# zengyan-97/X2-VLM

Measured on AMD Instinct MI355X. Metric: image-text pairs/sec (fwd+bwd) X2VLM-base 224px bs=64/GPU, higher is better.
Workload: dtype bf16

## Files before the change

### include/x2vlm_hip.h

```cpp
#ifndef X2VLM_HIP_H
#define X2VLM_HIP_H
#include <stdint.h>
#ifdef __cplusplus
extern "C" {
#endif

const char* x2_last_error(void);
int x2_abi_version(void);
int x2_device_cus(void);
int x2_tune(int key, int value);
int x2_tune_get(int key);

int x2_gemm_nt(const void* A, const void* B, void* C, int M, int N, int K, int lda, int ldb, int ldc,
               const float* bias, const float* gamma, const float* resid, int ldr, void* aux, int ldaux,
               int act, int out_f32, unsigned drop_thr16, unsigned drop_seed, float drop_scale, const unsigned* drop_epoch,
               const float* rowscale, float* colsum, void* stream);

int x2_gemm_nt_dgelu_colparts(const void* A, const void* B, void* C, int M, int N, int K, int lda, int ldb, int ldc,
                              const void* aux, int ldaux, float* colparts, int* nrows_out, void* stream);
int x2_gemm_nt_splitk(const void* A, const void* B, float* C, int M, int N, int K, int lda, int ldb, int ldc,
                      int slices, float* ws, long ws_floats, void* stream);

int x2_gemm_tn_grouped(const int64_t* problems, int count, int accumulate, int split, float* ws, long ws_floats,
                       void* stream);
int x2_tn_plan(const int64_t* shapes, int count, int cus, long ws_floats, int* windows, int max_windows, int* launches, int max_launches,
               int* n_windows, int* n_launches);
int x2_gemm_tn_queue(const int64_t* problems, int count, int accumulate, float* ws, long ws_floats, int first_launch, int n_launches,
                     void* stream);

typedef struct X2AttnArgs {
  const void *Q, *K, *V, *O, *dO;
  void *Out, *dQ, *dK, *dV, *dS;
  float *LSE, *Delta;
  long q_bs, q_rs, k_bs, k_rs, v_bs, v_rs, o_bs, o_rs;
  long dq_bs, dq_rs, dk_bs, dk_rs, dv_bs, dv_rs, do_bs, do_rs;
  int B, Bkv, H, Lq, Lk;
  float scale;
  const float* bias;  int bias_ld;
  const float* biasT; int biasT_ld;
  const float* mask;  int mask_ld;
  const int* kv_idx;
  const int* seq_off; const int* seq_ids;
  int ds_ld;
  unsigned drop_thr16, drop_seed; float drop_scale;
  int dbg;
  int head_dim;
  const unsigned* drop_epoch;
  int grid_nx, grid_ny, grid_nz, grid_map;
  int phase;
  float* ws; long ws_floats;
  float* colsum_ws;
} X2AttnArgs;
int x2_attn_fwd(const X2AttnArgs* args, void* stream);
int x2_attn_bwd(const X2AttnArgs* args, void* stream);
int x2_attn_bwd_one_pass(const X2AttnArgs* args);

int x2_layernorm_fwd(const float* x, const float* w, const float* b, void* y_bf16, float* y_f32, float* mean,
                     float* rstd, int rows, int D, float eps, int period, unsigned drop_thr16, unsigned drop_seed,
                     float drop_scale, const unsigned* drop_epoch, void* stream);
int x2_layernorm_bwd(const void* dy , int dy_is_bf16, const float* x, const float* mean, const float* rstd, const float* w,
                     const float* dres, float* dx, void* dx_bf16, float* dw, float* db, float* dcol, int rows, int D,
                     int period, unsigned in_thr16, unsigned in_seed, float in_scale, unsigned out_thr16,
                     unsigned out_seed, float out_scale, const unsigned* drop_epoch, float* ws ,
                     int defer, int post, const float* post_rowscale, void* stream);
int x2_colsum_bf16(const void* y, float* out, int M, int N, int ld, float* ws , int defer, void* stream);
int x2_reduce_partials(const float* part, int nblk, int nk, int width, float* o0, float* o1, float* o2, void* stream);
int x2_reduce_partials_multi(const int64_t* desc, int count, void* stream);
int x2_layerscale_finish(const int64_t* desc, int count, void* stream);
int x2_rowscale_cast_colsum(const float* dx, const float* rowscale, void* dx_bf16, float* colsum, int M, int D,
                            float* ws , int defer, void* stream);
int x2_cast_bf16(const float* src, void* dst, long n, void* stream);
int x2_cast_transpose_bf16(const float* src, void* dst, void* dstT, int R, int C, int ldt, void* stream);
int x2_cast_transpose_multi(const int64_t* desc, int count, void* stream);
int x2_copy_f32_multi(const int64_t* desc, int count, void* stream);
int x2_patchify(const float* image, void* cols, int B, int R, int ps, void* stream);
int x2_assemble_tokens(const float* patch, const float* cls, float* x, int B, int P, int D, void* stream);
int x2_assemble_tokens_bwd(const float* dx, void* dpatch_bf16, float* dcls, int B, int P, int D, void* stream);
int x2_pool_tokens(float* x, const float* w, int B, int P, int D, int bwd, void* stream);
int x2_relpos_bias(const float* table, const long* index, const long* indexT , float* bias, float* biasT, int N, int H, int ld, int ldT,
                   float scale, void* stream);
int x2_relpos_bias_bwd(const void* dS, const int* inv_off, const int* inv_pos, float* dtable, int B, int N, int H, int ld,
                       int T, float* ws, int slices, void* stream);

int x2_embed_fwd(const long* ids, const float* word, const float* pos, const float* type0, float* out, int R, int L,
                 int D, void* stream);
int x2_embed_bwd(const long* ids, const float* g, float* dword, float* dpos, float* dtype0, int R, int L, int D,
                 float* scratch, void* stream);
int x2_gather_rows(const float* src, const int* idx, float* dst, void* dst_bf16, int R, long len, void* stream);
int x2_scatter_rows(const float* src, const int* idx, float* dst, int R, int D, long len, void* stream);
int x2_linear_f32(const float* A, const float* B, float* C, const float* bias, const float* alpha_ptr, float alpha,
                  int M, int N, int K, long sam, long sak, long sbn, long sbk, long ldc, int accumulate,
                  int ksplit ,
                  float* ws , void* stream);
int x2_l2norm(const float* x, const float* dy, float* out, int R, int D, int bwd, void* stream);
int x2_ce_fwd(const float* logits, long ld, const long* labels, int R, int C, float* lse, float* loss_row, float* out2,
              void* stream);
int x2_ce_bwd(const float* logits, long ld, const long* labels, const float* lse, const float* g, const float* stat,
              float gscale, int R, int C, float* dl_f32, void* dl_bf16, long ldd, void* stream);
int x2_mlm_ce_fwd(const void* X, const void* E, const float* bias, const long* labels, int R, int Vp, int V, int Hd,
                  int ldx, int lde, float* part, float* zlab, void* stream);
int x2_ce_combine(const float* part, int chunks, const float* zlab, const long* labels, int R, float* lse, float* loss_row,
                  float* out2, void* stream);
int x2_mlm_ce_bwd(const void* X, const void* E, const float* bias, const long* labels, const float* lse, const float* g,
                  const float* stat, float gscale, int R, int Vp, int V, int Hd, int ldx, int lde, void* dl_bf16, long ldd,
                  void* stream);
int x2_mask_tokens(const long* text_ids, const long* text_atts, int B, int L, const unsigned char* is_subword, int vocab,
                   const unsigned* words, int words_ld, unsigned seed, const unsigned* epoch, double mask_prob, int max_masks,
                   double skipgram_prb, int skipgram_size, int mask_whole_word, long cls_id, long mask_id, long pad_id, long pad_mask,
                   long* text_ids_masked, long* masked_pos, long* masked_ids, void* stream);
int x2_sample_negatives(const float* sim, int n, const long* group, const float* u, int* out, void* stream);
int x2_additive_mask(const long* atts, float* out, int S, int L, int Lp, float neg, void* stream);
// ... 86 lines not shown
```

### x2-vlm_amd/_lib.py

```python
import contextlib
import ctypes as C
import os

import torch

_HERE = os.path.dirname(os.path.abspath(__file__))
LIB_PATH = os.environ.get("X2VLM_HIP_LIB") or os.path.join(_HERE, "libx2vlm_hip.so")

P, I, L, F, U = C.c_void_p, C.c_int, C.c_long, C.c_float, C.c_uint


class AttnArgs(C.Structure):
    _fields_ = [(n, P) for n in ("Q", "K", "V", "O", "dO", "Out", "dQ", "dK", "dV", "dS", "LSE", "Delta")] + \
               [(n, L) for n in ("q_bs", "q_rs", "k_bs", "k_rs", "v_bs", "v_rs", "o_bs", "o_rs",
                                 "dq_bs", "dq_rs", "dk_bs", "dk_rs", "dv_bs", "dv_rs", "do_bs", "do_rs")] + \
               [(n, I) for n in ("B", "Bkv", "H", "Lq", "Lk")] + [("scale", F)] + \
               [("bias", P), ("bias_ld", I), ("biasT", P), ("biasT_ld", I), ("mask", P), ("mask_ld", I),
                ("kv_idx", P), ("seq_off", P), ("seq_ids", P), ("ds_ld", I),
                ("drop_thr16", C.c_uint), ("drop_seed", C.c_uint), ("drop_scale", F), ("dbg", I), ("head_dim", I), ("drop_epoch", P),
                ("grid_nx", I), ("grid_ny", I), ("grid_nz", I), ("grid_map", I),
                ("phase", I), ("ws", P), ("ws_floats", L), ("colsum_ws", P)]


_SIGS = {
    "x2_gemm_nt": [P, P, P, I, I, I, I, I, I, P, P, P, I, P, I, I, I, U, U, F, P, P, P, P],
    "x2_gemm_nt_splitk": [P, P, P, I, I, I, I, I, I, I, P, L, P],
    "x2_gemm_nt_dgelu_colparts": [P, P, P, I, I, I, I, I, I, P, I, P, C.POINTER(I), P],
    "x2_gemm_tn_grouped": [P, I, I, I, P, L, P],
    "x2_gemm_tn_queue": [P, I, I, P, L, I, I, P],
    "x2_attn_fwd": [C.POINTER(AttnArgs), P],
    "x2_attn_bwd": [C.POINTER(AttnArgs), P],
    "x2_layernorm_fwd": [P, P, P, P, P, P, P, I, I, F, I, U, U, F, P, P],
    "x2_layernorm_bwd": [P, I, P, P, P, P, P, P, P, P, P, P, I, I, I, U, U, F, U, U, F, P, P, I, I, P, P],
    "x2_colsum_bf16": [P, P, I, I, I, P, I, P],
    "x2_reduce_partials": [P, I, I, I, P, P, P, P],
    "x2_reduce_partials_multi": [P, I, P],
    "x2_cast_transpose_multi": [P, I, P],
    "x2_copy_f32_multi": [P, I, P],
    "x2_layerscale_finish": [P, I, P],
    "x2_rowscale_cast_colsum": [P, P, P, P, I, I, P, I, P],
    "x2_cast_bf16": [P, P, L, P],
    "x2_cast_transpose_bf16": [P, P, P, I, I, I, P],
    "x2_patchify": [P, P, I, I, I, P],
    "x2_assemble_tokens": [P, P, P, I, I, I, P],
    "x2_assemble_tokens_bwd": [P, P, P, I, I, I, P],
    "x2_pool_tokens": [P, P, I, I, I, I, P],
    "x2_relpos_bias": [P, P, P, P, P, I, I, I, I, F, P],
    "x2_relpos_bias_bwd": [P, P, P, P, I, I, I, I, I, P, I, P],
    "x2_embed_fwd": [P, P, P, P, P, I, I, I, P],
    "x2_embed_bwd": [P, P, P, P, P, I, I, I, P, P],
    "x2_gather_rows": [P, P, P, P, I, L, P],
    "x2_scatter_rows": [P, P, P, I, I, L, P],
    "x2_linear_f32": [P, P, P, P, P, F, I, I, I, L, L, L, L, L, I, I, P, P],
    "x2_l2norm": [P, P, P, I, I, I, P],
    "x2_ce_fwd": [P, L, P, I, I, P, P, P, P],
    "x2_ce_bwd": [P, L, P, P, P, P, F, I, I, P, P, L, P],
    "x2_mlm_ce_fwd": [P, P, P, P, I, I, I, I, I, I, P, P, P],
    "x2_ce_combine": [P, I, P, P, I, P, P, P, P],
    "x2_mlm_ce_bwd": [P, P, P, P, P, P, P, F, I, I, I, I, I, I, P, L, P],
    "x2_sample_negatives": [P, I, P, P, P, P],
    "x2_mask_tokens": [P, P, I, I, P, I, P, I, U, P, C.c_double, I, C.c_double, I, I, L, L, L, L, P, P, P, P],
    "x2_additive_mask": [P, P, I, I, I, F, P],
    "x2_kv_csr": [P, I, I, P, P, P],
    "x2_tail_index": [P, P, P, P, I, I, I, I, P, P, P, P, P],
    "x2_droppath_rows": [P, U, P, I, I, I, P, P],
    "x2_frame_mean": [P, P, P, P, P, I, I, I, I, I, P],
    "x2_gelu_f32": [P, P, P, L, P],
    "x2_grad_norm": [P, I, I, F, P, P, P],
    "x2_adamw_multi": [P, I, I, P, P, I, F, F, F, P, P],
    "x2_colsum_f32": [P, P, I, I, P],
    "x2_attn_fwd_mask2d": [C.POINTER(AttnArgs), P, I, P],
    "x2_attn_bwd_mask2d": [C.POINTER(AttnArgs), P, I, P],
    "x2_additive_mask2d": [P, P, I, I, I, F, P],
    "x2_embed_fwd_pid": [P, P, P, P, P, P, I, I, P],
    "x2_embed_bwd_pid": [P, P, P, P, P, P, I, I, I, P, P],
    "x2_mlm_ls_fwd": [P, P, P, P, L, I, I, I, I, I, I, P, P, P, P, P],
    "x2_ls_combine": [P, P, I, P, P, P, P, I, I, L, F, P, P, P, P],
    "x2_mlm_ls_bwd": [P, P, P, P, P, P, P, P, F, F, L, I, I, I, I, I, I, P, L, P],
    "x2_attn_decode": [P, I, P, P, I, I, I, I, I, I, F, P],
    "x2_beam_gather": [P, P, P, I, I, I, I, I, P],
    "x2_logprob_topk": [P, I, I, I, P, I, I, I, I, I, I, P, P, P, P],
    "x2_answer_topk": [P, I, I, I, P, I, I, P, P, P],
    "x2_vqa_candidates": [P, P, P, I, I, I, I, L, P, P, P, P, I, P],
    "x2_vqa_rerank": [P, I, P, P, I, I, P, P, P, P],
    "x2_vqa_train_rows": [P, P, P, P, I, I, I, L, P, P, P, I, P, P],
    "x2_seq_loss_combine": [P, I, P, P, I, I, P, P, P, P, P],
    "x2_mlm_seq_bwd": [P, P, P, P, P, P, P, I, I, I, I, I, I, I, P, L, P],
    "x2_bbox_loss_fwd": [P, P, P, I, P, P, P],
    "x2_bbox_loss_bwd": [P, P, P, P, P, P, P, I, P, P],
    "x2_grounding_iou": [P, P, P, I, P, P, P],
    "x2_cls_tail_fwd": [P, I, P, P, P, P, P, I, I, I, F, P, P, P, P, P],
    "x2_cls_tail_bwd": [P, I, P, P, P, P, P, P, P, P, P, I, I, I, P, I, P, P, P, P, P],
    "x2_cls_accuracy": [P, P, I, I, P, P, P],
    "x2_lngelu_fwd": [P, I, P, P, I, I, F, P, I, P, P],
    "x2_lngelu_bwd": [P, I, P, I, P, P, P, I, I, P, I, P, P, P],
    "x2_soft_ce_fwd": [P, I, I, I, P, P, P, I, P, P, P, P],
    "x2_kl_ce_fwd": [P, I, P, I, I, I, P, P, P, P, P],
    "x2_soft_ce_bwd": [P, I, I, I, P, P, P, P, P, P, P, I, P, I, I, P],
    "x2_kl_ce_bwd": [P, I, P, I, I, I, P, P, P, P, I, P, I, I, P],
    "x2_cls_accuracy_rows": [P, I, P, I, I, P, P, P, P],
}
_COMM_SIGS = {
    "x2_comm_unique_id": [P],
    "x2_comm_init": [P, I, I, C.POINTER(P)],
    "x2_comm_info": [P, C.POINTER(I), C.POINTER(I)],
    "x2_comm_allreduce_bucket": [P, P, L, I, I, P, P],
    "x2_comm_allgather": [P, P, P, L, I, P, P],
    "x2_comm_broadcast": [P, P, L, I, I, P, P],
    "x2_comm_destroy": [P],
}
EXPORTS = sorted(list(_SIGS) + list(_COMM_SIGS) + ["x2_last_error", "x2_abi_version", "x2_device_cus", "x2_tune", "x2_tune_get",
                                                         "x2_attn_bwd_one_pass", "x2_tn_plan"])

_lib = None


class X2HipError(RuntimeError):
    pass


def lib():
    global _lib
    if _lib is None:
        if not os.path.exists(LIB_PATH):
            raise X2HipError("HIP extension %s not built: run `python -c 'import __graft_entry__ as g; g.build()'`"
                             % LIB_PATH)
        try:
            h = C.CDLL(LIB_PATH)
        except OSError as e:
            raise X2HipError("cannot load %s: %s" % (LIB_PATH, e))
        for name, sig in list(_SIGS.items()) + list(_COMM_SIGS.items()):
            fn = getattr(h, name)
            fn.argtypes, fn.restype = sig, I
        h.x2_last_error.restype = C.c_char_p
        h.x2_abi_version.restype = I
        h.x2_device_cus.restype = I
        h.x2_tune.argtypes, h.x2_tune.restype = [I, I], I
        h.x2_tune_get.argtypes, h.x2_tune_get.restype = [I], I
        h.x2_attn_bwd_one_pass.argtypes, h.x2_attn_bwd_one_pass.restype = [C.POINTER(AttnArgs)], I
        h.x2_tn_plan.argtypes, h.x2_tn_plan.restype = [P, I, I, L, P, I, P, I, C.POINTER(I), C.POINTER(I)], I
        for kv in filter(None, os.environ.get("X2_TUNE", "").split(",")):
            k, v = kv.split("=")
            set_tune(int(k), int(v), h)
        _lib = h
    return _lib


def set_tune(key, value, h=None):
    h = lib() if h is None else h
    if h.x2_tune(key, value) != 0:
        raise X2HipError("x2_tune(%d, %d): %s" % (key, value, h.x2_last_error().decode()))


@contextlib.contextmanager
def tuned(knobs):
    h = lib()
    with contextlib.ExitStack() as undo:
        for key, value in knobs.items():
            prev = h.x2_tune_get(key)
            if prev == -1:
                raise X2HipError("x2_tune_get(%d): no such key" % key)
            if prev != value:
                set_tune(key, value, h)
                undo.callback(set_tune, key, prev, h)
        yield


_get_device = torch._C._cuda_getDevice if hasattr(torch._C, "_cuda_getDevice") else None
_get_raw_stream = getattr(torch._C, "_cuda_getCurrentRawStream", None)


def raw_stream():
    return _get_raw_stream(_get_device())


def call(name, *args):
    h = _lib or lib()
    rc = getattr(h, name)(*args, _get_raw_stream(_get_device()))
    if rc != 0:
        raise X2HipError("%s failed (%d): %s" % (name, rc, h.x2_last_error().decode()))


def ptr(t):
    return None if t is None else t.data_ptr()
```

### x2-vlm_amd/csrc/gemm.hip

```cpp
#include "x2_common.h"
#include <algorithm>
#include <type_traits>
#include <vector>

#define BM 128
#define BN 128
#define BK 64
#define TILE_BYTES (128 * 128)
#define STAGE_BYTES (2 * TILE_BYTES)
#define GEMM_LDS_BYTES (2 * STAGE_BYTES)

struct GemmNT {
  const bf16_t* A; const bf16_t* B; void* C;
  const float* bias; const float* gamma; const float* resid; bf16_t* aux;
  int M, N, K;
  int lda, ldb, ldc, ldr, ldaux;
  int act;
  int out_f32;
  int group_m;
  DropSpec drop;
  const uint32_t* drop_epoch;
  const float* rowscale;
  float* colsum;
  int dbg;
// ... 1513 lines not shown
  const float* src = ws + (size_t)tile * 65536 + (size_t)e * 4;
  float4 o = *reinterpret_cast<const float4*>(src);
  for (int s_ = 1; s_ < split; ++s_) {
    const float4 v = *reinterpret_cast<const float4*>(src + (size_t)s_ * total_tiles * 65536);
    o.x += v.x; o.y += v.y; o.z += v.z; o.w += v.w;
  }
  if (n >= p.N || k >= p.K) return;
  float* dst = p.C + (size_t)n * p.ldc + k;
  if (g.accumulate) { const float4 c = *reinterpret_cast<float4*>(dst); o.x += c.x; o.y += c.y; o.z += c.z; o.w += c.w; }
  *reinterpret_cast<float4*>(dst) = o;
}

static int tn_parse(const char* who, const int64_t* q, int i, TNProblem& p) {
  p.A = (const bf16_t*)q[0]; p.B = (const bf16_t*)q[1]; p.C = (float*)q[2];
  p.Mc = (int)q[3]; p.N = (int)q[4]; p.K = (int)q[5]; p.lda = (int)q[6]; p.ldb = (int)q[7]; p.ldc = (int)q[8];
  p.n_ld = (int)q[9]; p.k_ld = (int)q[10];
  p.tile_begin = 0; p.tiles_k = 0; p.tile_first = 0;
  X2_REQUIRE(p.Mc > 0 && p.N > 0 && p.K > 0, "%s[%d]: empty problem", who, i);
  X2_REQUIRE(p.K % 4 == 0 && p.ldc % 4 == 0, "%s[%d]: K, ldc must be multiples of 4", who, i);
  X2_REQUIRE(p.lda % 8 == 0 && p.ldb % 8 == 0 && p.n_ld % 8 == 0 && p.k_ld % 8 == 0 && p.n_ld >= 8 && p.k_ld >= 8,
             "%s[%d]: rows must be 16-byte granular", who, i);
  X2_REQUIRE(p.n_ld <= p.lda && p.k_ld <= p.ldb, "%s[%d]: n_ld/k_ld exceed leading dims", who, i);
  return X2_OK;
}
static int tn_split_rule(int t, int min_steps, int cus, int split, bool have_ws, long ws_floats) {
  int sp = split;
  if (sp == 0) {
    double best = -1.0; sp = 1;
    for (int c = 1; c <= 4 && min_steps / c >= 16; ++c) {
      const long blocks = (long)t * c;
      const double fill = (double)blocks / (double)(((blocks + cus - 1) / cus) * cus);
      if (fill > best + 0.03) { best = fill; sp = c; }
    }
  }
  while (sp > 1 && (sp > min_steps || !have_ws || (long)sp * t * 65536 > ws_floats)) --sp;
  return sp;
}
static void tn256_launch(const GemmTNGroup& g, int t, int sp, float* ws, hipStream_t stream) {
  static bool attr = false;
  if (!attr) {
    (void)hipFuncSetAttribute(reinterpret_cast<const void*>(gemm_tn256_kernel<false>), hipFuncAttributeMaxDynamicSharedMemorySize, T2_LDS_BYTES);
    (void)hipFuncSetAttribute(reinterpret_cast<const void*>(gemm_tn256_kernel<true>), hipFuncAttributeMaxDynamicSharedMemorySize, T2_LDS_BYTES);
    attr = true;
  }
  bool ragged = false;
  for (int i = 0; i < g.count; ++i) ragged = ragged || (g.p[i].Mc % BK != 0);
  if (ragged) hipLaunchKernelGGL(gemm_tn256_kernel<true>, dim3(t, sp), dim3(512), T2_LDS_BYTES, stream, g, ws, t);
  else hipLaunchKernelGGL(gemm_tn256_kernel<false>, dim3(t, sp), dim3(512), T2_LDS_BYTES, stream, g, ws, t);
  if (sp > 1) hipLaunchKernelGGL(gemm_tn256_reduce_kernel, dim3(t * 64), dim3(256), 0, stream, g, ws, t, sp);
}

extern "C" int x2_gemm_tn_grouped(const int64_t* problems, int count, int accumulate, int split, float* ws, long ws_floats,
                                  void* stream) {
  X2_REQUIRE(count >= 1 && count <= 8, "x2_gemm_tn_grouped: count=%d not in [1,8]", count);
  X2_REQUIRE(split >= 0, "x2_gemm_tn_grouped: split=%d", split);
  GemmTNGroup g{}; g.count = count; g.accumulate = accumulate;
  int tiles256 = 0, min_steps = 1 << 30;
  bool big = g_tune[5] != 1;
  for (int i = 0; i < count; ++i) {
    TNProblem& p = g.p[i];
    if (int rc = tn_parse("x2_gemm_tn_grouped", problems + i * 11, i, p)) return rc;
    tiles256 += ((p.N + 255) / 256) * ((p.K + 255) / 256);
    const int steps_i = (p.Mc + BK - 1) / BK;
    min_steps = steps_i < min_steps ? steps_i : min_steps;
  }
  if (g_tune[5] != 2 && tiles256 < 24 && !(split > 1 && ws)) big = false;
  if (big) {
    int t = 0;
    for (int i = 0; i < count; ++i) { g.p[i].tile_begin = t; g.p[i].tiles_k = (g.p[i].K + 255) / 256; t += ((g.p[i].N + 255) / 256) * g.p[i].tiles_k; }
    const int sp = tn_split_rule(t, min_steps, x2_cus(), split, ws != nullptr, ws_floats);
    tn256_launch(g, t, sp, ws, (hipStream_t)stream);
    return x2_check_launch("x2_gemm_tn_grouped");
  }
  if (split == 0) split = 1;
  X2_REQUIRE(split == 1 || accumulate, "x2_gemm_tn_grouped: split>1 on the 128x128 kernel adds atomically: pass accumulate=1 and a defined C");
  int t = 0;
  for (int i = 0; i < count; ++i) { g.p[i].tile_begin = t; g.p[i].tiles_k = (g.p[i].K + 127) / 128; t += ((g.p[i].N + 127) / 128) * g.p[i].tiles_k; }
  hipLaunchKernelGGL(gemm_tn_kernel, dim3(t, split), dim3(256), GEMM_LDS_BYTES, (hipStream_t)stream, g);
  return x2_check_launch("x2_gemm_tn_grouped");
}

struct TNWindow { int launch, problem, first, tiles; };
struct TNPlan { std::vector<TNWindow> win; std::vector<int> split, remainder; };
static void tn_plan(const int64_t* shapes, int stride, int count, int cus, long ws_floats, TNPlan& plan) {
  std::vector<int> tiles(count), steps(count);
  long total = 0;
  for (int i = 0; i < count; ++i) {
    const int64_t* q = shapes + (size_t)i * stride;
    tiles[i] = (int)(((q[1] + 255) / 256) * ((q[2] + 255) / 256));
    steps[i] = (int)((q[0] + BK - 1) / BK);
    total += tiles[i];
  }
  const long main_tiles = total / cus * cus;
  int launch = -1;
  auto emit = [&](long from, long to, bool rem, bool dry) -> long {
    if (!dry) { ++launch; plan.split.push_back(1); plan.remainder.push_back(rem ? 1 : 0); }
    long begin = 0, pos = from;
    int entries = 0;
    for (int i = 0; i < count && pos < to && entries < TN_MAX_ENTRIES; begin += tiles[i], ++i) {
      if (pos >= begin + tiles[i]) continue;
      const int first = (int)(pos - begin), n = (int)std::min<long>(tiles[i] - first, to - pos);
      if (!dry) plan.win.push_back(TNWindow{launch, i, first, n});
      ++entries; pos += n;
    }
    return pos;
  };
  for (long pos = 0; pos < main_tiles;) {
    long end = emit(pos, main_tiles, false, true);
    if (end < main_tiles && end / cus * cus > pos) end = end / cus * cus;
    pos = emit(pos, end, false, false);
  }
  for (long pos = main_tiles; pos < total;) pos = emit(pos, total, true, false);
  for (int l = 0; l <= launch; ++l) {
    if (!plan.remainder[l]) continue;
    int t = 0, min_steps = 1 << 30;
    for (const TNWindow& w : plan.win) if (w.launch == l) { t += w.tiles; min_steps = std::min(min_steps, steps[w.problem]); }
    plan.split[l] = tn_split_rule(t, min_steps, cus, 0, ws_floats > 0, ws_floats);
  }
}

extern "C" int x2_tn_plan(const int64_t* shapes, int count, int cus, long ws_floats, int* windows, int max_windows, int* launches,
                          int max_launches, int* n_windows, int* n_launches) {
  X2_REQUIRE(shapes && count >= 1 && n_windows && n_launches, "x2_tn_plan: null argument or count=%d", count);
  for (int i = 0; i < count; ++i)
    X2_REQUIRE(shapes[3 * i] > 0 && shapes[3 * i + 1] > 0 && shapes[3 * i + 2] > 0 && shapes[3 * i] < (1L << 31) && shapes[3 * i + 1] < (1L << 24) &&
               shapes[3 * i + 2] < (1L << 24), "x2_tn_plan[%d]: Mc, N, K out of range", i);
  if (cus <= 0) cus = x2_cus();
  TNPlan plan;
  tn_plan(shapes, 3, count, cus, ws_floats, plan);
  *n_windows = (int)plan.win.size(); *n_launches = (int)plan.split.size();
  X2_REQUIRE((windows || max_windows == 0) && (launches || max_launches == 0), "x2_tn_plan: null output");
  if (max_windows == 0 && max_launches == 0) return X2_OK;
  X2_REQUIRE(*n_windows <= max_windows && *n_launches <= max_launches, "x2_tn_plan: %d windows, %d launches exceed the room given (%d, %d)",
             *n_windows, *n_launches, max_windows, max_launches);
  for (size_t w = 0; w < plan.win.size(); ++w) {
    windows[4 * w] = plan.win[w].launch; windows[4 * w + 1] = plan.win[w].problem; windows[4 * w + 2] = plan.win[w].first; windows[4 * w + 3] = plan.win[w].tiles;
  }
  for (size_t l = 0; l < plan.split.size(); ++l) { launches[2 * l] = plan.split[l]; launches[2 * l + 1] = plan.remainder[l]; }
  return X2_OK;
}

extern "C" int x2_gemm_tn_queue(const int64_t* problems, int count, int accumulate, float* ws, long ws_floats, int first_launch,
                                int n_launches, void* stream) {
  X2_REQUIRE(problems && count >= 1 && first_launch >= 0 && n_launches >= 0, "x2_gemm_tn_queue: count=%d first_launch=%d n_launches=%d", count,
             first_launch, n_launches);
  std::vector<TNProblem> pr(count);
  long tiles256 = 0;
  for (int i = 0; i < count; ++i) {
    if (int rc = tn_parse("x2_gemm_tn_queue", problems + (size_t)i * 11, i, pr[i])) return rc;
    tiles256 += (long)((pr[i].N + 255) / 256) * ((pr[i].K + 255) / 256);
  }
  if (g_tune[5] == 1 || (g_tune[5] != 2 && tiles256 < 24)) {
    X2_REQUIRE(first_launch == 0, "x2_gemm_tn_queue: first_launch=%d of a one-launch plan", first_launch);
    for (int i = 0; i < count; i += 8)
      if (int rc = x2_gemm_tn_grouped(problems + (size_t)i * 11, std::min(8, count - i), accumulate, 0, ws, ws_floats, stream)) return rc;
    return X2_OK;
  }
  if (!ws) ws_floats = 0;
  TNPlan plan;
  tn_plan(problems + 3, 11, count, x2_cus(), ws_floats, plan);
  const int nl = (int)plan.split.size();
  X2_REQUIRE(first_launch < nl, "x2_gemm_tn_queue: first_launch=%d of %d launches", first_launch, nl);
  const int end = n_launches == 0 ? nl : std::min(nl, first_launch + n_launches);
  size_t w = 0;
  for (int l = 0; l < end; ++l) {
    GemmTNGroup g{}; g.count = 0; g.accumulate = accumulate;
    int t = 0;
    for (; w < plan.win.size() && plan.win[w].launch == l; ++w) {
      TNProblem& p = g.p[g.count++];
      p = pr[plan.win[w].problem];
      p.tile_begin = t; p.tiles_k = (p.K + 255) / 256; p.tile_first = plan.win[w].first;
      t += plan.win[w].tiles;
    }
    if (l < first_launch) continue;
    tn256_launch(g, t, plan.split[l], ws, (hipStream_t)stream);
  }
  return x2_check_launch("x2_gemm_tn_queue");
}
```

### x2-vlm_amd/engine.py

```python
import itertools
import math
import weakref

import torch

from . import kernels as K
from ._lib import raw_stream

BF16, F32 = torch.bfloat16, torch.float32



_SERIAL = itertools.count(1)


def _tok(w):
    t = w.__dict__.get("_x2_serial")
    if t is None:
        t = w.__dict__["_x2_serial"] = next(_SERIAL)
    return t


class TScale:

# ... 166 lines not shown
        self.key = key

    @staticmethod
    def zero_all(arenas, extra=()):
        desc = [(0, g.flat.data_ptr(), g.nzero) for g in arenas if g.nzero] + [(0, t.data_ptr(), t.numel()) for t in extra]
        if not desc:
            return
        if arenas[0].flat.is_cuda if arenas else extra[0].is_cuda:
            K.copy_f32_multi(desc)
        else:
            for g in arenas:
                g.flat[:g.nzero].zero_()
            for t in extra:
                t.zero_()

    def __getitem__(self, name):
        return self.g[name]

    def alias(self, name, view):
        self.g[name] = view

    def publish(self, also_after=None):
        if GRAD_READY_HOOK is not None:
            GRAD_READY_HOOK(self.flat, self.key, also_after, self.params)

    def take(self, names):
        return [self.g.pop(n) for n in names]


class SideStream:

    def __init__(self):
        self.streams = {}
        self.held = {}
        self.enabled = True
        self.only_from = None

    @property
    def stream(self):
        key = raw_stream()
        if key not in self.streams:
            self.streams[key] = torch.cuda.Stream()
        return self.streams[key]

    def launch(self, fn, tensors):
        if not self.enabled or not torch.cuda.is_available() or (self.only_from is not None and raw_stream() != self.only_from):
            fn()
            return None
        side = self.stream
        ev = torch.cuda.Event()
        ev.record()
        side.wait_event(ev)
        done = torch.cuda.Event()
        with torch.cuda.stream(side):
            fn()
            done.record()
        self.held.setdefault(raw_stream(), []).append(tensors)
        return done

    def join(self):
        if self.enabled and torch.cuda.is_available():
            key = raw_stream()
            if key in self.streams and (self.only_from is None or key == self.only_from):
                torch.cuda.current_stream().wait_stream(self.streams[key])
            self.held.pop(key, None)


SIDE = SideStream()
AUX = SideStream()
AUX.enabled = False
AUX.auto = False


def _begin_layer_backward():
    K.DEFERRED = [] if torch.cuda.is_available() else None


class _LayerPairs:

    def __init__(self):
        self.pending = []
        self.extra = []
        self.fin = []

    def add(self, G, tn, param_only=(), finish=()):
        deferred, K.DEFERRED = K.DEFERRED, None
        if len(tn) > 4:
            self.flush()
            self._launch([(G, tn, deferred)], list(param_only), list(finish))
            return
        self.pending.append((G, tn, deferred))
        self.extra += list(param_only)
        self.fin += list(finish)
        if len(self.pending) == 2:
            self.flush()

    def flush(self):
        if self.pending:
            entries, self.pending = self.pending, []
            extra, self.extra = self.extra, []
            fin, self.fin = self.fin, []
            self._launch(entries, extra, fin)

    @staticmethod
    def _launch(entries, extra=(), fin=()):
        deferred = [d for _, _, ds in entries for d in (ds or ())]
        tn = [pr for _, t, _ in entries for pr in t]

        def work():
            if deferred:
                K.reduce_partials_multi(deferred)
            K.gemm_tn_grouped(tn)
            if fin:
                K.layerscale_finish(fin)
        if WGRAD_QUEUE is not None:
            tn_a = [tuple(pr[:2]) + (pr[2].detach(),) + tuple(pr[3:]) for pr in tn]
            def_a = [(ws, nblk, nk, width, tuple(None if o is None else o.detach() for o in outs)) for ws, nblk, nk, width, outs in deferred]
            fin_a = [tuple(t.detach() if (torch.is_tensor(t) and not isinstance(t, torch.nn.Parameter)) else t for t in it) for it in fin]
            pubs = [(G.flat, G.key, list(G.params)) for G, _, _ in entries]

            extra = list(extra)

            def pre():
                for fn in extra:
                    fn()
                if def_a:
                    K.reduce_partials_multi(def_a)

            def post():
                if fin_a:
                    K.layerscale_finish(fin_a)
                if GRAD_READY_HOOK is not None:
                    for flat, key, params in pubs:
                        GRAD_READY_HOOK(flat, key, None, params)

            def later():
                pre()
                K.gemm_tn_grouped(tn_a)
                post()
            later.pre, later.tn, later.post = pre, tn_a, post
            later.params = set(id(p_) for _, _, ps in pubs for p_ in ps)
            for fn in WGRAD_QUEUE:
                if getattr(fn, "params", set()) & later.params:
                    raise RuntimeError("engine.WGRAD_QUEUE: a layer ran twice in one pass; its weight gradients cannot be deferred "
                                       "(graph.SegmentedStep: defer_tail_wgrad, the deferred vision stages)")
            WGRAD_QUEUE.append(later)
            return
        assert not extra, "param_only closures are only collected while WGRAD_QUEUE is set"
        keep = [t for pr in tn for t in pr[:2]] + [G.flat for G, _, _ in entries] + [d[0] for d in deferred]
        done = SIDE.launch(work, keep)
        for G, _, _ in entries:
            G.publish(done)


def run_wgrad_queue(work):
    work = list(work or ())
    if len(work) < 2:
        for fn in work:
            fn()
        return
    for fn in work:
        assert fn.tn, "engine.run_wgrad_queue: a queued layer without weight-gradient problems"
        fn.pre()
    tn, ends = [], {}
    for fn in work:
        tn += fn.tn
        ends[len(tn) - 1] = fn.post
    K.gemm_tn_queue(tn, done=lambda i: ends.pop(i)() if i in ends else None)
    assert not ends, "engine.run_wgrad_queue: %d layers were never completed" % len(ends)


def _param_only(po, fn, src, dst):
    if WGRAD_QUEUE is not None:
        dst_a = dst.detach()
        po.append(lambda: fn(src, dst_a))
    else:
        fn(src, dst)


def _finish_layer_backward(G, tn):
    deferred, K.DEFERRED = K.DEFERRED, None
    _LayerPairs._launch([(G, tn, deferred)])


WGRAD_QUEUE = None
GRAD_READY_HOOK = None
STAGE_CALLS = {}


def _count_call(key):
    STAGE_CALLS[key] = STAGE_CALLS.get(key, 0) + 1


def _mask_pad(add_mask, Lk):
    S = add_mask.shape[0]
    out = torch.zeros(S, K.round_up(Lk, 64), device=add_mask.device, dtype=F32)
    out[:, :Lk] = add_mask
    return out



def vision_param_names(depth, lo=0, hi=None):
    hi = depth if hi is None else hi
    names = []
    if lo == 0:
        names += ["cls_token", "patch_embed.proj.weight", "patch_embed.proj.bias"]
    if hi == depth:
        names += ["fc_norm.weight", "fc_norm.bias"]
    for i in range(lo, hi):
        b = "blocks.%d." % i
        names += [b + s for s in ("gamma_1", "gamma_2", "norm1.weight", "norm1.bias", "attn.q_bias", "attn.v_bias",
                                  "attn.relative_position_bias_table", "attn.qkv.weight", "attn.proj.weight",
                                  "attn.proj.bias", "norm2.weight", "norm2.bias", "mlp.fc1.weight", "mlp.fc1.bias",
                                  "mlp.fc2.weight", "mlp.fc2.bias")]
    return names


class VisionEncoderFn(torch.autograd.Function):

    @staticmethod
    def forward(ctx, image, meta, *params):
        depth = meta["depth"]
        lo, hi = meta.get("lo", 0), meta.get("hi", depth)
        stem, head = lo == 0, hi == depth
        names = vision_param_names(depth, lo, hi)
        p = dict(zip(names, params))
        H = meta["heads"]
        if stem:
            B, R, ps = image.shape[0], image.shape[-1], meta["patch"]
            P_ = (R // ps) ** 2
            T = P_ + 1
            D = p["cls_token"].numel()
        else:
            B, T, D = image.shape
            P_ = T - 1
        M = B * T
        assert D == 64 * H, "vision width %d / %d heads: the attention kernels are built for head dim 64" % (D, H)
        scale = (D // H) ** -0.5
        BANK.prepare(([(p["patch_embed.proj.weight"],)] if stem else []) +
                     [(p["blocks.%d.%s.weight" % (i, n)],) for i in range(lo, hi) for n in ("attn.qkv", "mlp.fc1")] +
                     [(p["blocks.%d.%s.weight" % (i, n)], TScale(p["blocks.%d.%s" % (i, g_)])) for i in range(lo, hi)
                      for n, g_ in (("attn.proj", "gamma_1"), ("mlp.fc2", "gamma_2"))])
        BANK.prepare_vectors([(p["blocks.%d.attn.q_bias" % i], D, p["blocks.%d.attn.v_bias" % i]) for i in range(lo, hi)])
        cols = None
        if stem:
            cols = K.patchify(image.contiguous(), ps)
            wpe, _ = BANK.linear(p["patch_embed.proj.weight"])
            patch = K.gemm_nt(cols, wpe, bias=p["patch_embed.proj.bias"], out_dtype=F32)
            x = K.assemble_tokens(patch, p["cls_token"].reshape(-1), B, P_).view(M, D)
        else:
            x = image.contiguous().view(M, D)
        saved = []
        dpath = meta.get("drop_path")
        for i in range(lo, hi):
            b = "blocks.%d." % i
            rs1, rs2 = dpath[i] if dpath is not None else (None, None)
            h1, _, mean1, rstd1 = K.layernorm_fwd(x, p[b + "norm1.weight"], p[b + "norm1.bias"], meta["eps"])
            wqkv, _ = BANK.linear(p[b + "attn.qkv.weight"])
            qkv_bias = BANK.vector(p[b + "attn.q_bias"], D, p[b + "attn.v_bias"])
            qkv = K.gemm_nt(h1, wqkv, bias=qkv_bias)
            bias, biasT = K.relpos_bias(p[b + "attn.relative_position_bias_table"].detach(), meta["rel_index"], log2=True)
            att = torch.empty(M, D, device=x.device, dtype=BF16)
            lse = torch.empty(B * H * T, device=x.device, dtype=F32)
            K.attn_fwd(K.view3(qkv, B, T, 0), K.view3(qkv, B, T, D), K.view3(qkv, B, T, 2 * D), B, B, H, T, T, scale,
                       K.view3(att, B, T), lse, bias=bias, bias_log2=True)
# ... 693 lines not shown
```

### x2-vlm_amd/kernels.py

```python
import ctypes as C

import torch

from . import _lib
from ._lib import AttnArgs, call, ptr, raw_stream

BF16, F32 = torch.bfloat16, torch.float32


GEMM_TIMER = None


class _timed:

    def __init__(self, flops, name="gemm_nt"):
        self.flops = flops
        self.name = name

    def __enter__(self):
        if GEMM_TIMER is not None:
            self.a = torch.cuda.Event(enable_timing=True)
            self.b = torch.cuda.Event(enable_timing=True)
            self.a.record()

# ... 141 lines not shown
    if out is None:
        out = torch.empty(M, N, device=A.device, dtype=F32)
    assert out.shape == (M, N) and out.dtype == F32
    ws = workspace(A.device, min(32, max(1, K // 64)) * M * N)
    with _timed(2.0 * M * N * K):
        call("x2_gemm_nt_splitk", ptr(A), ptr(B), ptr(out), M, N, K, _rows(A), _rows(B), _rows(out), slices, ptr(ws), ws.numel())
    return out


def gemm_tn_grouped(problems, accumulate=False, split=0):
    rows = _tn_rows(problems)
    dev = problems[0][0].device
    for i in range(0, len(rows), 8):
        chunk = rows[i:i + 8]
        arr = (C.c_int64 * (11 * len(chunk)))(*[v for r in chunk for v in r])
        tiles256 = sum(((r[4] + 255) // 256) * ((r[5] + 255) // 256) for r in chunk)
        want = (split if split else 4) * tiles256 * 65536
        ws = workspace(dev, want) if split != 1 else None
        with _timed(sum(2.0 * r[3] * r[4] * r[5] for r in chunk), "gemm_tn"):
            call("x2_gemm_tn_grouped", arr, len(chunk), 1 if accumulate else 0, split, ptr(ws), 0 if ws is None else ws.numel())


_CUS = {}


def _device_cus(dev):
    if dev not in _CUS:
        _CUS[dev] = (_lib.lib().x2_device_cus() if dev.type == "cuda" else 0) or 256
    return _CUS[dev]


def _tn_rows(problems):
    rows = []
    for pr in problems:
        dY, X, dW = pr[:3]
        assert dY.dtype == BF16 and X.dtype == BF16 and dW.dtype == F32 and dY.shape[0] == X.shape[0]
        N, K = dW.shape
        n_ld, k_ld = (pr[3], pr[4]) if len(pr) == 5 else (dY.shape[1], X.shape[1])
        assert dY.shape[1] >= N or n_ld >= N
        rows.append([dY.data_ptr(), X.data_ptr(), dW.data_ptr(), dY.shape[0], N, K, _rows(dY), _rows(X), _rows(dW), n_ld, k_ld])
    return rows


def tn_plan(shapes, cus=0, ws_floats=0):
    flat = (C.c_int64 * (3 * len(shapes)))(*[int(v) for s in shapes for v in s])
    nw, nl = C.c_int(0), C.c_int(0)
    h = _lib.lib()

    def ask(*a):
        if h.x2_tn_plan(flat, len(shapes), cus, ws_floats, *a, C.byref(nw), C.byref(nl)) != 0:
            raise RuntimeError("x2_tn_plan: %s" % h.x2_last_error().decode())
    ask(None, 0, None, 0)
    win, lau = (C.c_int * (4 * nw.value))(), (C.c_int * (2 * nl.value))()
    ask(win, nw.value, lau, nl.value)
    return ([tuple(win[4 * i:4 * i + 4]) for i in range(nw.value)], [tuple(lau[2 * i:2 * i + 2]) for i in range(nl.value)])


def gemm_tn_queue(problems, accumulate=False, done=None):
    rows = _tn_rows(problems)
    dev = problems[0][0].device
    arr = (C.c_int64 * (11 * len(rows)))(*[v for r in rows for v in r])
    tiles = [((r[4] + 255) // 256) * ((r[5] + 255) // 256) for r in rows]
    want = 4 * min(sum(tiles), max(_device_cus(dev) - 1, 1)) * 65536
    ws = workspace(dev, want)
    acc = 1 if accumulate else 0
    flops = sum(2.0 * r[3] * r[4] * r[5] for r in rows)
    if done is None or sum(tiles) < 24 or _lib.lib().x2_tune_get(5) == 1:
        with _timed(flops, "gemm_tn"):
            call("x2_gemm_tn_queue", arr, len(rows), acc, ptr(ws), want, 0, 0)
        for i in range(len(rows) if done is not None else 0):
            done(i)
        return
    windows, launches = tn_plan([r[3:6] for r in rows], 0, want)
    last = {}
    for launch, prob, _first, _n in windows:
        last[prob] = launch
    nxt = 0
    for l in range(len(launches)):
        with _timed(flops / len(launches), "gemm_tn"):
            call("x2_gemm_tn_queue", arr, len(rows), acc, ptr(ws), want, l, 1)
        while nxt < len(rows) and last[nxt] == l:
            done(nxt)
            nxt += 1



def _attn_args(q, k, v, B, Bkv, H, Lq, Lk, scale, bias=None, biasT=None, mask=None, kv_idx=None, seq_off=None,
               seq_ids=None, drop=NO_DROP, head_dim=64, bias_log2=False):
    a = AttnArgs()
    a.Q, a.q_bs, a.q_rs = q
    a.K, a.k_bs, a.k_rs = k
    a.V, a.v_bs, a.v_rs = v
    a.B, a.Bkv, a.H, a.Lq, a.Lk, a.scale = B, Bkv, H, Lq, Lk, scale
    a.head_dim = head_dim
    a.dbg = 16 if bias_log2 else 0
    a.drop_thr16, a.drop_seed, a.drop_scale = drop[:3]
    a.drop_epoch = ptr(drop[3])
    if bias is not None:
        assert bias.dtype == F32 and bias.dim() == 3 and bias.is_contiguous()
        a.bias, a.bias_ld = bias.data_ptr(), bias.shape[2]
    if biasT is not None:
        assert biasT.dtype == F32 and biasT.dim() == 3 and biasT.is_contiguous()
        a.biasT, a.biasT_ld = biasT.data_ptr(), biasT.shape[2]
    if mask is not None:
        assert mask.dtype == F32 and mask.dim() == 2 and mask.is_contiguous() and mask.shape[0] == B
        a.mask, a.mask_ld = mask.data_ptr(), mask.shape[1]
    if kv_idx is not None:
        assert kv_idx.dtype == torch.int32 and kv_idx.numel() == B
        a.kv_idx = kv_idx.data_ptr()
    if seq_off is not None:
        assert seq_off.dtype == torch.int32 and seq_ids.dtype == torch.int32
        a.seq_off, a.seq_ids = seq_off.data_ptr(), seq_ids.data_ptr()
    return a


def view3(t, B, L, col0=0):
    assert t.dtype == BF16 and t.dim() == 2 and t.stride(1) == 1 and t.shape[0] == B * L
    return (t.data_ptr() + 2 * col0, L * t.stride(0), t.stride(0))


def attn_fwd(q, k, v, B, Bkv, H, Lq, Lk, scale, out, lse, **kw):
    a = _attn_args(q, k, v, B, Bkv, H, Lq, Lk, scale, **kw)
    a.Out, a.o_bs, a.o_rs = out
    assert lse.dtype == F32 and lse.numel() == B * H * Lq
    a.LSE = lse.data_ptr()
    call("x2_attn_fwd", C.byref(a))


def attn_bwd_form(Lq, Lk, shared_kv=False, dropout=False, workspace=False):
    a = AttnArgs()
    a.B = a.Bkv = a.H = 1
    a.Lq, a.Lk, a.head_dim, a.scale = Lq, Lk, 64, 0.125
    for f in ("q_bs", "q_rs", "k_bs", "k_rs", "v_bs", "v_rs", "o_bs", "o_rs", "dq_bs", "dq_rs", "dk_bs", "dk_rs", "dv_bs", "dv_rs", "do_bs", "do_rs"):
        setattr(a, f, 64)
    if shared_kv:
        a.kv_idx = a.seq_off = a.seq_ids = 8
    a.drop_thr16 = 1 if dropout else 0
    if workspace:
        a.ws, a.ws_floats = 8, ((Lq + 127) // 128) * 8192
    return _lib.lib().x2_attn_bwd_one_pass(C.byref(a))


def attn_bwd(q, k, v, o, do, B, Bkv, H, Lq, Lk, scale, lse, delta, dq, dk, dv, dS=None, phase=0, ask_form=False, colsum_ws=None, **kw):
    a = _attn_args(q, k, v, B, Bkv, H, Lq, Lk, scale, **kw)
    a.phase = phase
    a.O, a.o_bs, a.o_rs = o
    a.dO, a.do_bs, a.do_rs = do
    a.dQ, a.dq_bs, a.dq_rs = dq
    a.dK, a.dk_bs, a.dk_rs = dk
    a.dV, a.dv_bs, a.dv_rs = dv
    a.LSE, a.Delta = lse.data_ptr(), delta.data_ptr()
    if dS is not None:
        assert dS.dtype == BF16 and dS.is_contiguous() and dS.shape[:3] == (B, H, Lq)
        a.dS, a.ds_ld = dS.data_ptr(), dS.shape[3]
    if phase == 0 and Lq > 208 and Lk > 208 and a.kv_idx is None and not a.drop_thr16:
        ws = workspace(lse.device, B * H * ((Lq + 127) // 128) * 8192)
        a.ws, a.ws_floats = ws.data_ptr(), ws.numel()
    if ask_form:
        return _lib.lib().x2_attn_bwd_one_pass(C.byref(a))
    if colsum_ws is not None:
        assert colsum_ws.dtype == F32 and colsum_ws.is_contiguous() and colsum_ws.shape == (B, 2, H * 64)
        form = _lib.lib().x2_attn_bwd_one_pass(C.byref(a))
        if form in (1, 3):
            a.colsum_ws = colsum_ws.data_ptr()
        call("x2_attn_bwd", C.byref(a))
        return form
# ... 802 lines not shown
```

Measured before the change: 3037.

## Roll weight-gradient GEMM tiles across layers into CU-aligned side-stream launches

Replaces the per-layer-pair grouped weight-gradient GEMM launches with a rolling planner. Tiles from successive layers accumulate and are emitted as windowed launches whose tile counts are whole multiples of the CU count, with a remainder flush at the end. A new windowed TN GEMM entry point and a roll planner export support this, and layer gradients are published when their last window completes. The aim is to cut partial-wave tail inefficiency and launch count on the side stream. In exchange it adds host-side planning overhead per layer and delays gradient availability until a full wave fills.

```diff
diff --git a/include/x2vlm_hip.h b/include/x2vlm_hip.h
--- a/include/x2vlm_hip.h
+++ b/include/x2vlm_hip.h
@@ -27,6 +27,10 @@
                int* n_windows, int* n_launches);
 int x2_gemm_tn_queue(const int64_t* problems, int count, int accumulate, float* ws, long ws_floats, int first_launch, int n_launches,
                      void* stream);
+int x2_tn_roll(const int64_t* shapes, int count, int first_tile, int cus, long ws_floats, int flush, int* windows, int max_windows,
+               int* launches, int max_launches, int* n_windows, int* n_launches, int* last_launch, int* pending);
+int x2_gemm_tn_windows(const int64_t* problems, const int* windows, int count, int accumulate, int split, float* ws, long ws_floats,
+                       void* stream);
 
 typedef struct X2AttnArgs {
   const void *Q, *K, *V, *O, *dO;
diff --git a/x2-vlm_amd/_lib.py b/x2-vlm_amd/_lib.py
--- a/x2-vlm_amd/_lib.py
+++ b/x2-vlm_amd/_lib.py
@@ -28,6 +28,7 @@
     "x2_gemm_nt_dgelu_colparts": [P, P, P, I, I, I, I, I, I, P, I, P, C.POINTER(I), P],
     "x2_gemm_tn_grouped": [P, I, I, I, P, L, P],
     "x2_gemm_tn_queue": [P, I, I, P, L, I, I, P],
+    "x2_gemm_tn_windows": [P, P, I, I, I, P, L, P],
     "x2_attn_fwd": [C.POINTER(AttnArgs), P],
     "x2_attn_bwd": [C.POINTER(AttnArgs), P],
     "x2_layernorm_fwd": [P, P, P, P, P, P, P, I, I, F, I, U, U, F, P, P],
@@ -110,7 +111,7 @@
     "x2_comm_destroy": [P],
 }
 EXPORTS = sorted(list(_SIGS) + list(_COMM_SIGS) + ["x2_last_error", "x2_abi_version", "x2_device_cus", "x2_tune", "x2_tune_get",
-                                                         "x2_attn_bwd_one_pass", "x2_tn_plan"])
+                                                         "x2_attn_bwd_one_pass", "x2_tn_plan", "x2_tn_roll"])
 
 _lib = None
 
@@ -139,6 +140,7 @@
         h.x2_tune_get.argtypes, h.x2_tune_get.restype = [I], I
         h.x2_attn_bwd_one_pass.argtypes, h.x2_attn_bwd_one_pass.restype = [C.POINTER(AttnArgs)], I
         h.x2_tn_plan.argtypes, h.x2_tn_plan.restype = [P, I, I, L, P, I, P, I, C.POINTER(I), C.POINTER(I)], I
+        h.x2_tn_roll.argtypes, h.x2_tn_roll.restype = [P, I, I, I, L, I, P, I, P, I, C.POINTER(I), C.POINTER(I), P, P], I
         for kv in filter(None, os.environ.get("X2_TUNE", "").split(",")):
             k, v = kv.split("=")
             set_tune(int(k), int(v), h)
diff --git a/x2-vlm_amd/csrc/gemm.hip b/x2-vlm_amd/csrc/gemm.hip
--- a/x2-vlm_amd/csrc/gemm.hip
+++ b/x2-vlm_amd/csrc/gemm.hip
@@ -1619,7 +1619,7 @@
 
 struct TNWindow { int launch, problem, first, tiles; };
 struct TNPlan { std::vector<TNWindow> win; std::vector<int> split, remainder; };
-static void tn_plan(const int64_t* shapes, int stride, int count, int cus, long ws_floats, TNPlan& plan) {
+static void tn_plan(const int64_t* shapes, int stride, int count, int cus, long ws_floats, TNPlan& plan, long start = 0, bool flush = true) {
   std::vector<int> tiles(count), steps(count);
   long total = 0;
   for (int i = 0; i < count; ++i) {
@@ -1628,7 +1628,7 @@
     steps[i] = (int)((q[0] + BK - 1) / BK);
     total += tiles[i];
   }
-  const long main_tiles = total / cus * cus;
+  const long main_tiles = start + (total - start) / cus * cus;
   int launch = -1;
   auto emit = [&](long from, long to, bool rem, bool dry) -> long {
     if (!dry) { ++launch; plan.split.push_back(1); plan.remainder.push_back(rem ? 1 : 0); }
@@ -1642,12 +1642,13 @@
     }
     return pos;
   };
-  for (long pos = 0; pos < main_tiles;) {
+  for (long pos = start; pos < main_tiles;) {
     long end = emit(pos, main_tiles, false, true);
-    if (end < main_tiles && end / cus * cus > pos) end = end / cus * cus;
+    const long whole = start + (end - start) / cus * cus;
+    if (end < main_tiles && whole > pos) end = whole;
     pos = emit(pos, end, false, false);
   }
-  for (long pos = main_tiles; pos < total;) pos = emit(pos, total, true, false);
+  for (long pos = main_tiles; flush && pos < total;) pos = emit(pos, total, true, false);
   for (int l = 0; l <= launch; ++l) {
     if (!plan.remainder[l]) continue;
     int t = 0, min_steps = 1 << 30;
@@ -1714,3 +1715,62 @@
   }
   return x2_check_launch("x2_gemm_tn_queue");
 }
+
+extern "C" int x2_tn_roll(const int64_t* shapes, int count, int first_tile, int cus, long ws_floats, int flush, int* windows, int max_windows,
+                          int* launches, int max_launches, int* n_windows, int* n_launches, int* last_launch, int* pending) {
+  X2_REQUIRE(count >= 0 && (shapes || count == 0) && n_windows && n_launches && pending, "x2_tn_roll: null argument or count=%d", count);
+  X2_REQUIRE(count >= 1 || (flush && first_tile == 0), "x2_tn_roll: nothing to add (count=0, flush=%d, first_tile=%d)", flush, first_tile);
+  for (int i = 0; i < count; ++i)
+    X2_REQUIRE(shapes[3 * i] > 0 && shapes[3 * i + 1] > 0 && shapes[3 * i + 2] > 0 && shapes[3 * i] < (1L << 31) && shapes[3 * i + 1] < (1L << 24) &&
+               shapes[3 * i + 2] < (1L << 24), "x2_tn_roll[%d]: Mc, N, K out of range", i);
+  X2_REQUIRE(first_tile >= 0 && (count == 0 || first_tile < ((shapes[1] + 255) / 256) * ((shapes[2] + 255) / 256)),
+             "x2_tn_roll: first_tile=%d outside problem 0", first_tile);
+  if (cus <= 0) cus = x2_cus();
+  TNPlan plan;
+  if (count) tn_plan(shapes, 3, count, cus, ws_floats, plan, first_tile, flush != 0);
+  *n_windows = (int)plan.win.size(); *n_launches = (int)plan.split.size();
+  X2_REQUIRE((windows || max_windows == 0) && (launches || max_launches == 0), "x2_tn_roll: null output");
+  X2_REQUIRE(*n_windows <= max_windows && *n_launches <= max_launches, "x2_tn_roll: %d windows, %d launches exceed the room given (%d, %d)",
+             *n_windows, *n_launches, max_windows, max_launches);
+  for (size_t w = 0; w < plan.win.size(); ++w) {
+    windows[4 * w] = plan.win[w].launch; windows[4 * w + 1] = plan.win[w].problem; windows[4 * w + 2] = plan.win[w].first; windows[4 * w + 3] = plan.win[w].tiles;
+  }
+  for (size_t l = 0; l < plan.split.size(); ++l) { launches[2 * l] = plan.split[l]; launches[2 * l + 1] = plan.remainder[l]; }
+  int at = 0, tile = first_tile;
+  for (int i = 0; i < count && last_launch; ++i) last_launch[i] = -1;
+  for (const TNWindow& w : plan.win) {
+    at = w.problem; tile = w.first + w.tiles;
+    if (tile == (int)(((shapes[3 * at + 1] + 255) / 256) * ((shapes[3 * at + 2] + 255) / 256))) {
+      if (last_launch) last_launch[at] = w.launch;
+      ++at; tile = 0;
+    }
+  }
+  pending[0] = at; pending[1] = at < count ? tile : 0;
+  return X2_OK;
+}
+
+extern "C" int x2_gemm_tn_windows(const int64_t* problems, const int* windows, int count, int accumulate, int split, float* ws, long ws_floats,
+                                  void* stream) {
+  X2_REQUIRE(problems && windows && count >= 1 && count <= TN_MAX_ENTRIES, "x2_gemm_tn_windows: null argument or count=%d not in [1,%d]", count,
+             TN_MAX_ENTRIES);
+  X2_REQUIRE(split >= 1 && split <= 4, "x2_gemm_tn_windows: split=%d not in [1,4]", split);
+  GemmTNGroup g{}; g.count = count; g.accumulate = accumulate;
+  long t = 0;
+  for (int i = 0; i < count; ++i) {
+    TNProblem& p = g.p[i];
+    if (int rc = tn_parse("x2_gemm_tn_windows", problems + (size_t)i * 11, i, p)) return rc;
+    p.tiles_k = (p.K + 255) / 256;
+    const long grid = (long)((p.N + 255) / 256) * p.tiles_k;
+    const int first = windows[2 * i], n = windows[2 * i + 1];
+    X2_REQUIRE(first >= 0 && n >= 1 && (long)first + n <= grid, "x2_gemm_tn_windows[%d]: window (%d, %d) outside the problem's %ld tiles", i, first,
+               n, grid);
+    X2_REQUIRE((p.Mc + BK - 1) / BK >= split, "x2_gemm_tn_windows[%d]: %d slices of %d steps", i, split, (p.Mc + BK - 1) / BK);
+    p.tile_begin = (int)t; p.tile_first = first;
+    t += n;
+    X2_REQUIRE(t < (1L << 24), "x2_gemm_tn_windows: more than 2^24 tiles in one launch");
+  }
+  X2_REQUIRE(split == 1 || (ws && (long)split * t * 65536 <= ws_floats), "x2_gemm_tn_windows: %d slices of %ld tiles need %ld workspace floats (%ld given)",
+             split, t, (long)split * t * 65536, ws ? ws_floats : 0L);
+  tn256_launch(g, (int)t, split, ws, (hipStream_t)stream);
+  return x2_check_launch("x2_gemm_tn_windows");
+}
diff --git a/x2-vlm_amd/engine.py b/x2-vlm_amd/engine.py
--- a/x2-vlm_amd/engine.py
+++ b/x2-vlm_amd/engine.py
@@ -272,9 +272,23 @@
         self.pending = []
         self.extra = []
         self.fin = []
+        self.roll = None
+        self.probs = {}
+        self.layers = []
 
     def add(self, G, tn, param_only=(), finish=()):
         deferred, K.DEFERRED = K.DEFERRED, None
+        if WGRAD_QUEUE is None:
+            assert not param_only, "param_only closures are only collected while WGRAD_QUEUE is set"
+            assert tn, "a layer without weight-gradient problems"
+            if self.roll is None:
+                self.roll = K.TNRoll()
+            n0 = self.roll.base + len(self.roll.shapes)
+            for j, pr in enumerate(tn):
+                self.probs[n0 + j] = pr
+            self.layers.append([G, n0, n0 + len(tn) - 1, list(deferred or ()), list(finish)])
+            self._enqueue(*self.roll.add([(pr[0].shape[0],) + tuple(pr[2].shape) for pr in tn]))
+            return
         if len(tn) > 4:
             self.flush()
             self._launch([(G, tn, deferred)], list(param_only), list(finish))
@@ -291,56 +305,73 @@
             extra, self.extra = self.extra, []
             fin, self.fin = self.fin, []
             self._launch(entries, extra, fin)
+        if self.roll is not None and self.roll.shapes:
+            self._enqueue(*self.roll.flush(4 * self.roll.pending_tiles() * 65536))
+            assert not self.layers and not self.probs and not self.roll.shapes, "engine._LayerPairs: tiles left behind a flush"
+
+    def _enqueue(self, launches, last):
+        for number, split, _rem, wins in launches:
+            entries = [(self.probs[pid], first, n) for pid, first, n in wins]
+            top = wins[-1][0]
+            reds = []
+            for layer in self.layers:
+                if layer[1] <= top and layer[3]:
+                    reds += layer[3]
+                    layer[3] = None
+            done = [layer for layer in self.layers if last.get(layer[2]) == number]
+            fin = [it for layer in done for it in layer[4]]
+
+            def work():
+                if reds:
+                    K.reduce_partials_multi(reds)
+                K.gemm_tn_windows(entries, split)
+                if fin:
+                    K.layerscale_finish(fin)
+            keep = [t for pr, _, _ in entries for t in pr[:2]] + [layer[0].flat for layer in self.layers if layer[1] <= top] + [d[0] for d in reds]
+            ev = SIDE.launch(work, keep)
+            for pid, lnum in last.items():
+                if lnum == number:
+                    del self.probs[pid]
+            for layer in done:
+                self.layers.remove(layer)
+                layer[0].publish(ev)
 
     @staticmethod
     def _launch(entries, extra=(), fin=()):
         deferred = [d for _, _, ds in entries for d in (ds or ())]
         tn = [pr for _, t, _ in entries for pr in t]
-
-        def work():
-            if deferred:
-                K.reduce_partials_multi(deferred)
-            K.gemm_tn_grouped(tn)
-            if fin:
-                K.layerscale_finish(fin)
-        if WGRAD_QUEUE is not None:
-            tn_a = [tuple(pr[:2]) + (pr[2].detach(),) + tuple(pr[3:]) for pr in tn]
-            def_a = [(ws, nblk, nk, width, tuple(None if o is None else o.detach() for o in outs)) for ws, nblk, nk, width, outs in deferred]
-            fin_a = [tuple(t.detach() if (torch.is_tensor(t) and not isinstance(t, torch.nn.Parameter)) else t for t in it) for it in fin]
-            pubs = [(G.flat, G.key, list(G.params)) for G, _, _ in entries]
-
-            extra = list(extra)
-
-            def pre():
-                for fn in extra:
-                    fn()
-                if def_a:
-                    K.reduce_partials_multi(def_a)
-
-            def post():
-                if fin_a:
-                    K.layerscale_finish(fin_a)
-                if GRAD_READY_HOOK is not None:
-                    for flat, key, params in pubs:
-                        GRAD_READY_HOOK(flat, key, None, params)
-
-            def later():
-                pre()
-                K.gemm_tn_grouped(tn_a)
-                post()
-            later.pre, later.tn, later.post = pre, tn_a, post
-            later.params = set(id(p_) for _, _, ps in pubs for p_ in ps)
-            for fn in WGRAD_QUEUE:
-                if getattr(fn, "params", set()) & later.params:
-                    raise RuntimeError("engine.WGRAD_QUEUE: a layer ran twice in one pass; its weight gradients cannot be deferred "
-                                       "(graph.SegmentedStep: defer_tail_wgrad, the deferred vision stages)")
-            WGRAD_QUEUE.append(later)
-            return
-        assert not extra, "param_only closures are only collected while WGRAD_QUEUE is set"
-        keep = [t for pr in tn for t in pr[:2]] + [G.flat for G, _, _ in entries] + [d[0] for d in deferred]
-        done = SIDE.launch(work, keep)
-        for G, _, _ in entries:
-            G.publish(done)
+        assert WGRAD_QUEUE is not None, "engine._LayerPairs: closures are collected only while WGRAD_QUEUE is set"
+        tn_a = [tuple(pr[:2]) + (pr[2].detach(),) + tuple(pr[3:]) for pr in tn]
+        def_a = [(ws, nblk, nk, width, tuple(None if o is None else o.detach() for o in outs)) for ws, nblk, nk, width, outs in deferred]
+        fin_a = [tuple(t.detach() if (torch.is_tensor(t) and not isinstance(t, torch.nn.Parameter)) else t for t in it) for it in fin]
+        pubs = [(G.flat, G.key, list(G.params)) for G, _, _ in entries]
+
+        extra = list(extra)
+
+        def pre():
+            for fn in extra:
+                fn()
+            if def_a:
+                K.reduce_partials_multi(def_a)
+
+        def post():
+            if fin_a:
+                K.layerscale_finish(fin_a)
+            if GRAD_READY_HOOK is not None:
+                for flat, key, params in pubs:
+                    GRAD_READY_HOOK(flat, key, None, params)
+
+        def later():
+            pre()
+            K.gemm_tn_grouped(tn_a)
+            post()
+        later.pre, later.tn, later.post = pre, tn_a, post
+        later.params = set(id(p_) for _, _, ps in pubs for p_ in ps)
+        for fn in WGRAD_QUEUE:
+            if getattr(fn, "params", set()) & later.params:
+                raise RuntimeError("engine.WGRAD_QUEUE: a layer ran twice in one pass; its weight gradients cannot be deferred "
+                                   "(graph.SegmentedStep: defer_tail_wgrad, the deferred vision stages)")
+        WGRAD_QUEUE.append(later)
 
 
 def run_wgrad_queue(work):
@@ -366,11 +397,6 @@
         po.append(lambda: fn(src, dst_a))
     else:
         fn(src, dst)
-
-
-def _finish_layer_backward(G, tn):
-    deferred, K.DEFERRED = K.DEFERRED, None
-    _LayerPairs._launch([(G, tn, deferred)])
 
 
 WGRAD_QUEUE = None
diff --git a/x2-vlm_amd/kernels.py b/x2-vlm_amd/kernels.py
--- a/x2-vlm_amd/kernels.py
+++ b/x2-vlm_amd/kernels.py
@@ -247,6 +247,59 @@
         while nxt < len(rows) and last[nxt] == l:
             done(nxt)
             nxt += 1
+
+
+class TNRoll:
+
+    def __init__(self, cus=0):
+        self.cus = cus
+        self.shapes = []
+        self.base = 0
+        self.first = 0
+        self.launches = 0
+
+    @staticmethod
+    def tiles(shape):
+        return ((shape[1] + 255) // 256) * ((shape[2] + 255) // 256)
+
+    def pending_tiles(self):
+        return sum(self.tiles(s) for s in self.shapes) - self.first
+
+    def add(self, shapes, flush=False, ws_floats=0):
+        self.shapes += [tuple(int(v) for v in s) for s in shapes]
+        n = len(self.shapes)
+        if n == 0:
+            return [], {}
+        flat = (C.c_int64 * (3 * n))(*[v for s in self.shapes for v in s])
+        room = 2 * n + 4
+        win, lau, last, pend = (C.c_int * (4 * room))(), (C.c_int * (2 * room))(), (C.c_int * n)(), (C.c_int * 2)()
+        nw, nl = C.c_int(0), C.c_int(0)
+        h = _lib.lib()
+        if h.x2_tn_roll(flat, n, self.first, self.cus, ws_floats, 1 if flush else 0, win, room, lau, room, C.byref(nw), C.byref(nl), last, pend) != 0:
+            del self.shapes[n - len(shapes):]
+            raise RuntimeError("x2_tn_roll: %s" % h.x2_last_error().decode())
+        out = [(self.launches + l, lau[2 * l], lau[2 * l + 1], []) for l in range(nl.value)]
+        for w in range(nw.value):
+            out[win[4 * w]][3].append((self.base + win[4 * w + 1], win[4 * w + 2], win[4 * w + 3]))
+        done = {self.base + i: self.launches + last[i] for i in range(n) if last[i] >= 0}
+        self.launches += nl.value
+        self.base, self.first = self.base + pend[0], pend[1]
+        del self.shapes[:pend[0]]
+        return out, done
+
+    def flush(self, ws_floats=0):
+        return self.add([], True, ws_floats)
+
+
+def gemm_tn_windows(entries, split=1, accumulate=False):
+    rows = _tn_rows([e[0] for e in entries])
+    arr = (C.c_int64 * (11 * len(rows)))(*[v for r in rows for v in r])
+    win = (C.c_int * (2 * len(rows)))(*[int(v) for e in entries for v in e[1:3]])
+    want = split * sum(e[2] for e in entries) * 65536 if split > 1 else 0
+    ws = workspace(entries[0][0][0].device, want) if want else None
+    flops = sum(2.0 * r[3] * r[4] * r[5] * e[2] / TNRoll.tiles(r[3:6]) for r, e in zip(rows, entries))
+    with _timed(flops, "gemm_tn"):
+        call("x2_gemm_tn_windows", arr, win, len(rows), 1 if accumulate else 0, split, ptr(ws), want)
 
 
 
```

Result: no change. 3033 (-0.1%).
